# OpenResearchInstitute/opv-cxx-demod

Hardware: AMD Instinct MI355X
Metric: IQ Msamples/s demod+Viterbi (×real-time @2.168MSPS); BER vs ref (higher is better)
Workload: dtype f64; 1 GPU; configs[3]: 64 concurrent IQ streams/GPU x 1000 frames, -s semantics, amp 2000, f0 -2000..+2000 Hz across the 64 streams of a shard (SURVEY.md §8d C4: edge streams on the AFC clamp, outside the +/-1530 Hz search span), Eb/N0 16 dB; streams_per_gpu=64, parallelism=streams sharded 64/GPU, no data-path collective

## Files before the change

### opv-cxx-demod_amd/csrc/k_frontend.hip

```cpp
#include <hip/hip_runtime.h>
#include <math.h>

#include <type_traits>

#include "opv_device.h"

namespace {

constexpr double kPi = 3.14159265358979323846;
constexpr double kTwoPi = 2.0 * kPi;
constexpr double kFs = 2168000.0;
constexpr double kSymRate = 2168000.0 / 40.0;
constexpr double kDeltaPerHz = kTwoPi / kFs;

constexpr uint32_t kTile = OPV_TILE_SAMPLES;
constexpr uint32_t kRing = 2 * kTile;
constexpr uint32_t kRingBytes = kRing * 4;
constexpr uint32_t kGuardBytes = 16;
constexpr uint32_t kBack = 11;
constexpr uint32_t kAhead = 56;
static_assert((kRing & (kRing - 1)) == 0, "ring must be a power of two");

constexpr uint32_t kTabOff = kRingBytes + kGuardBytes;
static_assert(kTabOff % 16 == 0, "16-byte LDS alignment");

typedef __attribute__((address_space(1))) double gdouble;
typedef __attribute__((address_space(1))) unsigned char gbyte;

__device__ inline int dlo(double v) { return __double2loint(v); }
__device__ inline int dhi(double v) { return __double2hiint(v); }
__device__ inline double mkd(int hi, int lo) { return __hiloint2double(hi, lo); }

__device__ inline double swap32_add(double a, double b) {
    auto lo = __builtin_amdgcn_permlane32_swap((unsigned)dlo(a), (unsigned)dlo(b), false, false);
    auto hi = __builtin_amdgcn_permlane32_swap((unsigned)dhi(a), (unsigned)dhi(b), false, false);
    return mkd((int)hi[0], (int)lo[0]) + mkd((int)hi[1], (int)lo[1]);
}
__device__ inline double swap16_add(double a, double b) {
    auto lo = __builtin_amdgcn_permlane16_swap((unsigned)dlo(a), (unsigned)dlo(b), false, false);
    auto hi = __builtin_amdgcn_permlane16_swap((unsigned)dhi(a), (unsigned)dhi(b), false, false);
    return mkd((int)hi[0], (int)lo[0]) + mkd((int)hi[1], (int)lo[1]);
}
template <int N>
__device__ inline double row_bcast(double old, double v) { return __builtin_amdgcn_update_dpp(old, v, 0x150 + N, 0xF, 0xF, false); }
__device__ inline uint32_t uni(uint32_t v) { return (uint32_t)__builtin_amdgcn_readfirstlane((int)v); }
__device__ inline double readlane_d(double v, int l) {
    return mkd(__builtin_amdgcn_readlane(dhi(v), l), __builtin_amdgcn_readlane(dlo(v), l));
}
__device__ inline bool uni_lt(double a, double b) { return __builtin_amdgcn_fcmp(a, b, 4 ) != 0ull; }
__device__ inline bool uni_eq(double a, double b) { return __builtin_amdgcn_fcmp(a, b, 1 ) != 0ull; }
// ... 45 lines not shown
    th -= kTwoPi * rint(th / kTwoPi);
    double sn, cs;
    sincos(th, &sn, &cs);
    const unsigned q = (unsigned)((dom1 ? (4u - (unsigned)(ksym & 3u)) : (unsigned)(ksym & 3u)) & 3u);
    double er2 = cs, ei2 = sn;
    if (q == 1u) { er2 = -sn; ei2 = cs; }
    else if (q == 2u) { er2 = -cs; ei2 = -sn; }
    else if (q == 3u) { er2 = sn; ei2 = -cs; }
    double vr = dr, vi = di;
    if (dom_zero) {
        const double jr = dom1 ? pi : -pi, ji = dom1 ? -pr : pr;
        vr = jr * prv.x40c - ji * prv.x40s;
        vi = jr * prv.x40s + ji * prv.x40c;
    }
    const double qr = vr * er2 + vi * ei2;
    const double qi = vi * er2 - vr * ei2;
    return make_double2((qr < 0.0 && qi < 0.0) ? kPi : 0.0, tie);
}

}

#include "opv_atan2.h"

template <int WPB>
__device__ __forceinline__ void msk_frontend_body(OpvStream* __restrict__ streams, OpvGlobalCfg cfg, int n_streams,
                                                  unsigned char* lds_all) {
    const int lane = threadIdx.x & 63;
    const int wave = WPB == 1 ? 0 : __builtin_amdgcn_readfirstlane((int)(threadIdx.x >> 6));
    const int sidx = (int)blockIdx.x * WPB + wave;
    const uint64_t dbg_t0 = __builtin_amdgcn_s_memtime(), dbg_r0 = __builtin_amdgcn_s_memrealtime();

    unsigned char* const lds = lds_all + wave * kTabOff;
    const unsigned char* ringb = lds;
    double* atab = reinterpret_cast<double*>(lds_all + WPB * kTabOff);
    if (sidx >= n_streams) return;
    OpvStream& st = streams[sidx];

    const int jsamp = lane - (lane >> 4) - ((lane & 15) == 15 ? 1 : 0);
    const double kf = (double)(jsamp - 10);
    const double kfs = kf * kDeltaPerHz;
    double wr[15], wi[15];
    {
        const int row = lane >> 4, t = lane & 15, u = t & 7;
        const bool is_p = u >= 6, imag = t >= 8;
        const int gate = (u < 2 || is_p) ? 1 : ((u & 1) ? 2 : 0);
        const bool tone2 = is_p ? false : (u < 2 ? u == 1 : u >= 4);
#pragma unroll
        for (int n = 0; n < 15; ++n) {
            const int i = 15 * row + n - 10 * gate;
            double sn, cs;
            sincospi((double)i / 80.0, &sn, &cs);
            const bool in = i >= 0 && i < 40;
            const double a = in ? cs : 0.0, b = in ? -sn : 0.0;
            double r_, i_;
            if (is_p) { r_ = (t == 6) ? a : (t == 15 ? b : 0.0); i_ = (t == 7) ? b : (t == 14 ? a : 0.0); }
            else if (!imag) { r_ = a; i_ = tone2 ? -b : b; }
            else { r_ = tone2 ? b : -b; i_ = a; }
// ... 15 lines not shown
    asm volatile("" : "+v"(kc_halfpi), "+v"(kc_32), "+v"(kc_m1_32), "+v"(kc_gain));
    const double kc_nfomax = __builtin_canonicalize(-kc_fomax), kc_ntfmax = __builtin_canonicalize(-kc_tfmax);
    kc_fomax = __builtin_canonicalize(kc_fomax);
    kc_tfmax = __builtin_canonicalize(kc_tfmax);
    double sx = 1.0, nsg = 1.0;
    asm volatile("" : "+v"(sx), "+v"(nsg));

    double fo = st.freq_offset, tf = st.timing_freq, mu = st.mu;
    PrevSums qp{st.p1r, st.p1i, st.p2r, st.p2i, st.x40c, st.x40s}, qq{0, 0, 0, 0, 1, 0};
    double fo_sum = st.fo_sum;
    uint32_t origin = uni((uint32_t)st.origin);
    const uint32_t n_avail = uni((uint32_t)st.n_avail);
    uint64_t n_soft = st.n_soft, total_samples = st.total_samples;
    uint32_t n_chunks = uni(st.n_chunks);
    int tail_done = (int)uni((uint32_t)st.tail_done);
    const int eof = (int)uni((uint32_t)st.eof);
    int overflow = (int)uni((uint32_t)st.overflow), stalled = 0;
    uint32_t edge_ties = uni(st.edge_ties);
    const uint64_t cap_soft = st.cap_soft;
    if (cap_soft > (1ull << 28)) overflow = 1;
    uint64_t soft_keep = st.trk_next >= 24 ? st.trk_next - 24 : 0;
    if (st.trk_state != 0 && st.trk_anchor < soft_keep) soft_keep = st.trk_anchor;
    const uint32_t soft_bmask = (uint32_t)(cap_soft * 8u - 1u) & ~7u;
    gbyte* const soft_base = (gbyte*)st.soft;
    const gbyte* iq_bytes = (const gbyte*)st.iq;
    const uint64_t n_bytes = (uint64_t)n_avail * 4u;

    auto glds16 = [&](const gbyte* gsrc, uint32_t lds_byte) {
        unsigned keep;
        asm volatile("s_mov_b32 %0, m0\n\ts_mov_b32 m0, %2\n\ts_nop 0\n\tglobal_load_lds_dwordx4 %1, off\n\ts_mov_b32 m0, %0"
                     : "=&s"(keep)
                     : "v"(gsrc), "s"(uni(lds_byte))
                     : "memory");
    };
    const uint32_t lds_base = uni((uint32_t)(uintptr_t)(__attribute__((address_space(3))) unsigned char*)lds);
    auto issue_tile = [&](uint32_t t) {
        const uint64_t base = (uint64_t)t * OPV_TILE_BYTES;
        const uint32_t slot = (t & 1u) * OPV_TILE_BYTES;
#pragma unroll
        for (int r = 0; r < 8; ++r) {
            const uint32_t in_tile = (uint32_t)r * 1024u + (uint32_t)lane * 16u;
            const uint64_t off = base + in_tile;
            if (off + 16u <= n_bytes) glds16(iq_bytes + off, lds_base + slot + (uint32_t)r * 1024u);
            else if (off < n_bytes) {
                for (uint32_t j = 0; off + 4u * j < n_bytes; ++j)
                    *reinterpret_cast<int*>(lds + slot + in_tile + 4u * j) = *reinterpret_cast<const __attribute__((address_space(1))) int*>(iq_bytes + off + 4u * j);
            }
        }
        if ((t & 1u) == 0u && lane == 0) {
            if (base + 16u <= n_bytes) glds16(iq_bytes + base, lds_base + kRingBytes);
            else
                for (uint32_t j = 0; base + 4u * j < n_bytes && j < 4u; ++j)
                    *reinterpret_cast<int*>(lds + kRingBytes + 4u * j) = *reinterpret_cast<const __attribute__((address_space(1))) int*>(iq_bytes + base + 4u * j);
        }
    };
    uint32_t t_lo = (origin >= kBack ? origin - kBack : 0u) / kTile;
    issue_tile(t_lo);
    issue_tile(t_lo + 1u);
    __builtin_amdgcn_s_waitcnt(0x0F70);
    bool evt_issue = true;
    uint32_t next_evt = (t_lo + 1u) * kTile + kBack;

    for (;;) {
        const uint32_t remaining = n_avail - origin;
        uint32_t N;
        bool last = false;
        if (cfg.streaming) {
            if (remaining >= OPV_CHUNK) N = OPV_CHUNK;
            else if (eof && !tail_done && remaining > 0) { N = remaining; last = true; }
            else { if (eof) tail_done = 1; break; }
        } else {
            if (!eof || tail_done) break;
            N = n_avail;
            last = true;
        }
        if (overflow) break;
        if ((n_soft - soft_keep) + (uint64_t)(N / 38u + 2u) > cap_soft) { stalled = 1; break; }

        const double Nd = (double)N;
        double pos = mu;
        const uint32_t soft_off0 = ((uint32_t)n_soft * 8u) & soft_bmask;
        uint32_t soft_off = soft_off0;
        asm volatile("" : "+v"(soft_off));

        auto housekeeping = [&](double at) {
            const uint32_t b = uni((uint32_t)at);
            const uint32_t gb = origin + b;
            while (gb >= next_evt) {
                if (evt_issue) {
                    issue_tile(t_lo + 2u);
                    ++t_lo;
                    evt_issue = false;
                    next_evt = (t_lo + 1u) * kTile - kAhead;
                } else {
                    __builtin_amdgcn_s_waitcnt(0x0F70);
                    evt_issue = true;
                    next_evt = (t_lo + 1u) * kTile + kBack;
                }
            }
            const int lim1 = (int)(next_evt - gb) - 2, lim2 = (int)N - 52 - (int)b;
            int lim = lim1 < lim2 ? lim1 : lim2;
            if (lim < 0) lim = 0;
            return ((uint32_t)lim * 1560u) >> 16;
        };

        int w0 = 0, w1 = 0;
        double f = 0.0;
        uint32_t tap_byte = 0;
        auto fetch_addr = [&](double at, bool clamp0) {
            double p = at + kf;
            if (clamp0) p = fmax(p, 0.0);
            const int idx = (int)p;
            f = __builtin_amdgcn_fract(p);
            tap_byte = (((uint32_t)idx + origin) << 2) & (kRingBytes - 4u);
        };
        auto fetch_read = [&]() {
            const int* tap = reinterpret_cast<const int*>(ringb + tap_byte);
            w0 = tap[0];
            w1 = tap[1];
        };
        auto fetch = [&](double at, bool clamp0) {
            fetch_addr(at, clamp0);
            fetch_read();
        };

        auto symbol_r = [&](auto tag, PrevSums& cur, const PrevSums& prv) {
            constexpr bool kFirst = decltype(tag)::first;
            constexpr bool kWide = decltype(tag)::wide;
            double xs, xc;
            if constexpr (kWide) {
                if (__builtin_expect(uni_lt(2000.0, fabs(fo)), 0)) sincos(kfs * fo, &xs, &xc);
                else expj_small(kfs, fo, sck, xs, xc);
            } else {
                expj_small(kfs, fo, sck, xs, xc);
            }
            __builtin_amdgcn_sched_barrier(0);
            const uint32_t my_soft_off = soft_off;
            uint32_t soft_off_next = soft_off + 8u;
            asm volatile("" : "+v"(soft_off_next));
            __builtin_amdgcn_sched_barrier(0);
            const int s0r = (int)(short)(w0 & 0xFFFF), s0i = w0 >> 16;
            const int d_r = (int)(short)(w1 & 0xFFFF) - s0r, d_i = (w1 >> 16) - s0i;
            const double lr = fma(f, (double)d_r, (double)s0r);
            const double li = fma(f, (double)d_i, (double)s0i);
            const double zr = fma(lr, xc, li * xs);
            const double zi = fma(li, xc, -(lr * xs));
            __builtin_amdgcn_sched_barrier(0);

            double acc0, acc1, v, t;
#define OPV_RB(N) "v_fmac_f64_dpp %[a0], %[zr], %[r" #N "] row_newbcast:" #N " row_mask:0xf bank_mask:0xf\n\t" \
                  "v_fmac_f64_dpp %[a1], %[zi], %[i" #N "] row_newbcast:" #N " row_mask:0xf bank_mask:0xf\n\t"
            asm("v_mov_b64 %[a0], 0\n\tv_mov_b64 %[a1], 0\n\t" OPV_RB(0) OPV_RB(1) OPV_RB(2) OPV_RB(3) OPV_RB(4) OPV_RB(5) OPV_RB(6) OPV_RB(7)
                : [a0] "=&v"(acc0), [a1] "=&v"(acc1)
                : [zr] "v"(zr), [zi] "v"(zi), [r0] "v"(wr[0]), [i0] "v"(wi[0]), [r1] "v"(wr[1]), [i1] "v"(wi[1]), [r2] "v"(wr[2]), [i2] "v"(wi[2]),
                  [r3] "v"(wr[3]), [i3] "v"(wi[3]), [r4] "v"(wr[4]), [i4] "v"(wi[4]), [r5] "v"(wr[5]), [i5] "v"(wi[5]),
                  [r6] "v"(wr[6]), [i6] "v"(wi[6]), [r7] "v"(wr[7]), [i7] "v"(wi[7]));
            __builtin_amdgcn_sched_barrier(0);
            soft_off = soft_off_next & soft_bmask;
            asm volatile("" : "+v"(soft_off));
            __builtin_amdgcn_sched_barrier(0);
            asm(OPV_RB(8) OPV_RB(9) OPV_RB(10) OPV_RB(11) OPV_RB(12) OPV_RB(13) OPV_RB(14)
                "v_add_f64 %[v], %[a0], %[a1]\n\t"
                "v_mov_b64 %[t], %[v]"
                : [a0] "+v"(acc0), [a1] "+v"(acc1), [v] "=&v"(v), [t] "=&v"(t)
                : [zr] "v"(zr), [zi] "v"(zi), [r8] "v"(wr[8]), [i8] "v"(wi[8]), [r9] "v"(wr[9]), [i9] "v"(wi[9]), [r10] "v"(wr[10]), [i10] "v"(wi[10]),
                  [r11] "v"(wr[11]), [i11] "v"(wi[11]), [r12] "v"(wr[12]), [i12] "v"(wi[12]), [r13] "v"(wr[13]), [i13] "v"(wi[13]),
                  [r14] "v"(wr[14]), [i14] "v"(wi[14]));
// ... 35 lines not shown
            if constexpr (!kFirst) {
                const double dr = fma(sg, P2o, P1o), di = fma(-sg, P4o, P3o);
                const double prs = fma(sg, prv.a, prv.b), pis = fma(sg, prv.c, -prv.d);
                const double ar = fma(dr, prs, di * pis), ai = fma(di, prs, -(dr * pis));
                cy = fma(ar, prv.x40c, ai * prv.x40s);
                cx = fma(ar, prv.x40s, -(ai * prv.x40c));
                __builtin_amdgcn_sched_barrier(0);
                ee = row_bcast<2>(sq, seln); el = row_bcast<3>(shv, seln);
                __builtin_amdgcn_sched_barrier(0);
                sx = mkd((dhi(cx) & (int)0x80000000) | (dhi(sx) & 0x7fffffff), dlo(sx));
                asm volatile("" : "+v"(sx));
                sum = fabs(cx) + fabs(cy); dif = fabs(cy) - fabs(cx);
                dm_ = sum + kc_tiny;
                if constexpr (WPB == 1) {
                    zmask = __builtin_amdgcn_fcmp(sum, 0.0, 1 );
                    asm volatile("" : "+s"(zmask));
                }
            } else {
                ee = row_bcast<2>(sq, seln); el = row_bcast<3>(shv, seln);
            }
            const double den = el + ee + kc_eps;

            double ted, h = 0;
            [[maybe_unused]] double2 c01{0, 0}, c23{0, 0}, c45{0, 0};
            if constexpr (kFirst) {
                double y = __builtin_amdgcn_rcp(den);
                const double num = el - ee;
                y = fma(fma(-den, y, 1.0), y, y);
                y = fma(fma(-den, y, 1.0), y, y);
                ted = num * y;
                ted = fma(fma(-den, ted, num), y, ted);
            } else {
                const double dm = dm_;
                const double tt = den * dm;
                double y = __builtin_amdgcn_rcp(tt);
                const double num = el - ee;
                y = fma(fma(-tt, y, 1.0), y, y);
                const double iden = y * dm, idm = y * den;
                const double ratio = dif * idm;
                const double kt = fma(ratio, kc_64, kc_magic);
                h = ratio;
                const unsigned char* rowb = reinterpret_cast<const unsigned char*>(atab) + ((unsigned)dlo(kt) << 5);
                const double2* trow = reinterpret_cast<const double2*>(rowb);
                c23 = trow[1]; c01 = trow[0];
                ted = num * iden;
                ted = fma(fma(-den, ted, num), iden, ted);
            }
            __builtin_amdgcn_sched_barrier(0);
            tf = clampd(fma(kc_beta, ted, tf), kc_ntfmax, kc_tfmax);
            const double adj = fma(kc_alpha, ted, tf);
            pos += 40.0 + adj;
            fetch_addr(pos, false);
            __builtin_amdgcn_sched_barrier(0);
            fetch_read();
            __builtin_amdgcn_sched_barrier(0);
            *(gdouble*)(soft_base + my_soft_off) = soft;
            if constexpr (!kFirst) {
                const double pd_off = fma(-sx, kc_halfpi, kc_halfpi);
                __builtin_amdgcn_sched_barrier(0);
                __builtin_amdgcn_s_waitcnt(0xC17F);
                __builtin_amdgcn_sched_barrier(0);
                pd = fma(c23.y, h, c23.x);
                pd = fma(pd, h, c01.y);
                pd = fma(pd, h, c01.x);
                pd = fma(sx, pd, pd_off);
                pd = mkd((dhi(pd) & 0x7fffffff) | (dhi(cy) & (int)0x80000000), dlo(pd));
                if (__builtin_expect(WPB == 1 ? zmask != 0ull : uni_eq(sum, 0.0), 0)) {
                    const double dr = fma(sg, P2o, P1o), di = fma(-sg, P4o, P3o);
                    const double2 sp = silence_pd(dr, di, prv, soft < 0.0, fo_sum, n_soft + (((my_soft_off - soft_off0) & soft_bmask) >> 3),
                                                  P1o, P2o, P3o, P4o);
                    pd = sp.x;
                    edge_ties += uni((uint32_t)sp.y);
                }
                const double fo_new = fma(kc_gain, pd, fo);
                asm("v_max_f64 %0, %1, %2\n\tv_min_f64 %0, %0, %3" : "=&v"(fo) : "v"(fo_new), "v"(kc_nfomax), "v"(kc_fomax));
            }
            fo_sum = fo_sum_next;
            cur.a = P1o; cur.b = P2o; cur.c = P3o; cur.d = P4o;
        };

        auto sym = [&](auto tag, PrevSums& cur, const PrevSums& prv) { symbol_r(tag, cur, prv); };

        if (uni_lt(pos + 40.0 + 10.0, Nd)) {
            (void)housekeeping(pos);
            fetch(pos, true);
            sym(TagFirst{}, qp, qp);
            if (__builtin_expect(uni_lt(2000.0, fabs(fo)), 0) && uni_lt(pos + 40.0 + 10.0, Nd)) {
                (void)housekeeping(pos);
                fetch(pos, false);
                sym(TagSecond{}, qq, qp);
                qp = qq;
            }
            while (uni_lt(pos + 40.0 + 10.0, Nd)) {
                uint32_t pairs = uni(housekeeping(pos)) >> 1;
                fetch(pos, false);
                for (uint32_t quads = pairs >> 1; quads != 0u; --quads) {
                    sym(TagSteady{}, qq, qp);
                    sym(TagSteady{}, qp, qq);
                    sym(TagSteady{}, qq, qp);
                    sym(TagSteady{}, qp, qq);
                }
                pairs &= 1u;
                for (; pairs != 0u; --pairs) {
                    sym(TagSteady{}, qq, qp);
                    sym(TagSteady{}, qp, qq);
                }
                sym(TagSteady{}, qq, qp);
                qp = qq;
            }
        }

        const uint32_t nsym_call = ((soft_off - soft_off0) & soft_bmask) >> 3;
        const uint32_t used = uni((uint32_t)pos);
        mu = pos - (double)used;
        const uint32_t leftover = N - used;
        if (lane == 0) {
            double* c = st.chunk_log + 5 * (size_t)(n_chunks % st.cap_chunks);
            c[0] = fo;
            c[1] = tf; c[2] = mu; c[3] = (double)leftover; c[4] = (double)nsym_call;
        }
        ++n_chunks;
        n_soft += nsym_call;
        total_samples += N;
        origin += (leftover > 0u && leftover < N) ? used : N;
        if (last) { tail_done = 1; break; }
    }

    if (lane == 0) {
        st.freq_offset = fo;
        st.p1r = qp.a; st.p1i = qp.b; st.p2r = qp.c; st.p2i = qp.d; st.x40c = qp.x40c; st.x40s = qp.x40s;
        st.fo_sum = fo_sum;
        st.edge_ties = edge_ties;
        st.timing_freq = tf; st.mu = mu;
        st.origin = origin; st.n_soft = n_soft; st.total_samples = total_samples;
        st.n_chunks = n_chunks; st.tail_done = tail_done; st.overflow = overflow;
        st.stalled = stalled;
        unsigned hw, xcc;
        asm volatile("s_getreg_b32 %0, hwreg(HW_REG_HW_ID)" : "=s"(hw));
        asm volatile("s_getreg_b32 %0, hwreg(HW_REG_XCC_ID)" : "=s"(xcc));
        st.dbg_hw_id = hw; st.dbg_xcc_id = xcc;
        st.dbg_cycles = __builtin_amdgcn_s_memtime() - dbg_t0;
        st.dbg_ticks = __builtin_amdgcn_s_memrealtime() - dbg_r0;
    }
}

constexpr uint32_t kAtanQBytes = 1025 * 32;
template <int NT>
__device__ __forceinline__ void load_atan_table_q(unsigned char* lds_tab) {
    double* atab = reinterpret_cast<double*>(lds_tab);
    for (int i = threadIdx.x; i < 1025 * 4; i += NT) atab[i] = (&kOpvAtanTabQ3R[0][0])[i];
}
extern "C" __global__ __launch_bounds__(64) void k_msk_frontend_rb(OpvStream* __restrict__ streams, OpvGlobalCfg cfg,
                                                                    int n_streams) {
    __shared__ __attribute__((aligned(16))) unsigned char lds_all[kTabOff + kAtanQBytes];
    load_atan_table_q<64>(lds_all + kTabOff);
    __syncthreads();
    msk_frontend_body<1>(streams, cfg, n_streams, lds_all);
}
extern "C" __global__ __launch_bounds__(256) void k_msk_frontend_rb_wg4(OpvStream* __restrict__ streams, OpvGlobalCfg cfg,
                                                                         int n_streams) {
    __shared__ __attribute__((aligned(16))) unsigned char lds_all[4 * kTabOff + kAtanQBytes];
    load_atan_table_q<256>(lds_all + 4 * kTabOff);
    __syncthreads();
    msk_frontend_body<4>(streams, cfg, n_streams, lds_all);
}
```

### opv-cxx-demod_amd/csrc/opv_capi.hip

```cpp
#include <hip/hip_runtime.h>
#include <dlfcn.h>

#include <atomic>

#include <climits>
#include <cstddef>
#include <cmath>
#include <cstdio>
#include <cstdlib>
#include <cstring>
#include <new>
#include <string>
#include <thread>
#include <vector>

#include "../../include/opv_demod.h"
#include "opv_device.h"
#include "opv_offset_host.h"
#include "opv_tx_internal.h"

extern "C" __global__ void k_offset_search(OpvStream*, OpvGlobalCfg, const double*, uint32_t*);
extern "C" __global__ void k_tie_collect(const OpvStream*, const uint32_t*, uint32_t, uint32_t, uint32_t, OpvTieStage*);
extern "C" __global__ void k_tie_apply(OpvStream*, const OpvTieStage*, uint32_t, int);
extern "C" __global__ void k_msk_frontend_rb(OpvStream*, OpvGlobalCfg, int);
// ... 159 lines not shown
    static constexpr int kInSlots = 4;
    StreamIn* h_in = nullptr;
    hipEvent_t in_ev[kInSlots] = {};
    int* h_stall = nullptr;
    hipEvent_t done_ev = nullptr;
    unsigned round_no = 0;
    std::vector<OpvStream> mirror;
    std::vector<OpvStream> initial;
    std::vector<HostStream> hs;
    double* d_soft = nullptr;
    OpvFrameRec* d_frec = nullptr;
    OpvEventRec* d_events = nullptr;
    double* d_chunks = nullptr;
    uint8_t* d_frames = nullptr;
    int32_t* d_metrics = nullptr;
    double* d_fscale = nullptr;
    int32_t* d_counts = nullptr;
    double* d_offs_wtab = nullptr;
    uint32_t* d_tie_list = nullptr;
    bool host_ties = false;
    bool tx_trust_libm = false;
    bool push_gather = true;
    uint32_t push_gather_blocks = 32;
    struct TieWork {
        OpvTieStage* stage = nullptr;
        uint32_t slots = 0;
        std::atomic<uint64_t> decided{0};
        std::atomic<uint64_t> left{0};
    } tie;
    std::vector<int> search_now;
    void* h_bulk_tab = nullptr;
    size_t bulk_tab_bytes = 0;
    bool push_pending = false;
    hipEvent_t push_ev = nullptr;
    uint64_t cap_soft = 0;
    uint32_t cap_frames = 0, cap_events = 0, cap_chunks = 0;
    bool mirror_valid = false;
    bool maybe_stalled = false;
    double* d_tx_ckpt = nullptr;
    size_t tx_ckpt_cap = 0, tx_ckpt_have = 0;
    double* d_tx_phases = nullptr;
    size_t tx_phases_cap = 0, tx_phases_have = 0;
    uint8_t* d_tx_frames = nullptr;
    uint8_t* d_tx_codes = nullptr;
    uint8_t* d_tx_fpar = nullptr;
    size_t tx_frames_cap = 0;
// ... 78 lines not shown
}

extern "C" const char* opv_last_error(void) { return g_err.c_str(); }
extern "C" int opv_abi_version(void) { return OPV_ABI_VERSION; }

extern "C" int opv_create(opv_ctx** out, int n_streams, const opv_cfg* cfg) {
    if (!out || !cfg || n_streams <= 0 || cfg->max_samples == 0) return fail(OPV_EINVAL, "opv_create: bad arguments");
    if (cfg->max_samples >= (1ull << 31)) return fail(OPV_EINVAL, "opv_create: max_samples must be < 2^31");
    if ((cfg->have_init_offset && !std::isfinite(cfg->init_offset_hz)) || !std::isfinite(cfg->afc_alpha) || (cfg->coherent && !std::isfinite(cfg->pll_bw_hz)))
        return fail(OPV_EINVAL, "opv_create: init_offset_hz / afc_alpha / pll_bw_hz must be finite");
    int ndev = 0;
    if (hipGetDeviceCount(&ndev) != hipSuccess || ndev <= 0) return fail(OPV_ENODEV, "no HIP device visible");
    if (cfg->device < 0 || cfg->device >= ndev) return fail(OPV_ENODEV, "opv_cfg.device out of range");
    HIPCHK(hipSetDevice(cfg->device));
    hipDeviceProp_t prop;
    HIPCHK(hipGetDeviceProperties(&prop, cfg->device));
    if (std::strncmp(prop.gcnArchName, "gfx950", 6) != 0)
        return fail(OPV_ENODEV, "device is not gfx950 (MI355X); this library carries gfx950 code objects only");

    opv_ctx* c = new (std::nothrow) opv_ctx();
    if (!c) return fail(OPV_ENOMEM, "host allocation failed");
    c->n_streams = n_streams;
    c->cfg = *cfg;
    c->hs.resize(n_streams);
    c->mirror.resize(n_streams);

    const uint64_t M = cfg->max_samples;
    c->cap_soft = 1;
    while (c->cap_soft < M / 38 + 4096) c->cap_soft <<= 1;
    c->cap_frames = (uint32_t)(M / (uint64_t)(OPV_FSYMS * 38) + 4);
    c->cap_events = 4 * c->cap_frames + 64;
    c->cap_chunks = (uint32_t)(M / 80000 + 4);

    auto cleanup = [&](int code) { opv_destroy(c); return code; };
#define HIPCHK_C(expr)                                                        \
    do {                                                                      \
        hipError_t _e = (expr);                                               \
        if (_e != hipSuccess) return cleanup(fail(_e == hipErrorOutOfMemory ? OPV_ENOMEM : OPV_EHIP, #expr, _e)); \
    } while (0)

    HIPCHK_C(hipStreamCreateWithFlags(&c->stream, hipStreamNonBlocking));
    {
        int least = 0, greatest = 0;
        if (hipDeviceGetStreamPriorityRange(&least, &greatest) != hipSuccess ||
            hipStreamCreateWithPriority(&c->copy_stream, hipStreamNonBlocking, greatest) != hipSuccess) {
            (void)hipGetLastError();
// ... 15 lines not shown
    HIPCHK_C(hipMalloc(&c->d_chunks, sizeof(double) * 5 * c->cap_chunks * S));
    HIPCHK_C(hipMalloc(&c->d_frames, (size_t)OPV_FB * c->cap_frames * S));
    HIPCHK_C(hipMalloc(&c->d_metrics, sizeof(int32_t) * c->cap_frames * S));
    HIPCHK_C(hipMalloc(&c->d_fscale, sizeof(double) * c->cap_frames * S));
    HIPCHK_C(hipMalloc(&c->d_counts, sizeof(int32_t) * S));
    {
        std::vector<double> w((size_t)OPV_SPS * 2 * OPV_OFFS_TERMS);
        for (int i = 0; i < OPV_SPS; ++i) {
            const double u = (double)i - 19.5, cs = std::cos(M_PI * i / 80.0), sn = std::sin(M_PI * i / 80.0);
            double t = 1.0;
            for (int k = 0; k < OPV_OFFS_TERMS; ++k) {
                w[((size_t)i * 2 + 0) * OPV_OFFS_TERMS + k] = cs * t;
                w[((size_t)i * 2 + 1) * OPV_OFFS_TERMS + k] = sn * t;
                t = t * u / (double)(k + 1);
            }
        }
        HIPCHK_C(hipMalloc(&c->d_offs_wtab, sizeof(double) * w.size()));
        HIPCHK_C(hipMemcpy(c->d_offs_wtab, w.data(), sizeof(double) * w.size(), hipMemcpyHostToDevice));
    }
    c->host_ties = opv_offset_host_libm_matches_reference() && !std::getenv("OPV_OFFSET_DISTRUST_LIBM");
    c->tx_trust_libm = libm_flat_tops_as_assumed() && !std::getenv("OPV_TX_DISTRUST_LIBM");
    c->push_gather = !std::getenv("OPV_PUSH_NO_GATHER");
    if (const char* e = std::getenv("OPV_PUSH_GATHER_BLOCKS")) { const int v = atoi(e); if (v > 0) c->push_gather_blocks = (uint32_t)v; }
    if (c->host_ties) {
        HIPCHK_C(hipMalloc(&c->d_tie_list, sizeof(uint32_t) * (S + 1)));
        c->tie.slots = (uint32_t)(S < (size_t)OPV_TIE_SLOTS_MAX ? S : (size_t)OPV_TIE_SLOTS_MAX);
        if (hipHostMalloc((void**)&c->tie.stage, offsetof(OpvTieStage, slot) + sizeof(OpvTieSlot) * c->tie.slots, hipHostMallocDefault) != hipSuccess) {
            (void)hipGetLastError();
            c->tie.stage = nullptr;
            c->host_ties = false;
        } else {
            c->tie.stage->n = c->tie.stage->listed = c->tie.stage->beyond = 0;
        }
    }
    HIPCHK_C(hipMemsetAsync(c->d_frames, 0, (size_t)OPV_FB * c->cap_frames * S, c->stream));
    HIPCHK_C(hipMemsetAsync(c->d_counts, 0, sizeof(int32_t) * S, c->stream));
    k_fill_i32<<<256, 256, 0, c->stream>>>(c->d_metrics, INT32_MIN, (size_t)c->cap_frames * S);

    for (size_t i = 0; i < S; ++i) {
        OpvStream s;
        std::memset(&s, 0, sizeof s);
        s.soft = c->d_soft + c->cap_soft * i;
        s.cap_soft = c->cap_soft;
        s.frec = c->d_frec + (size_t)c->cap_frames * i;
        s.events = c->d_events + (size_t)c->cap_events * i;
        s.chunk_log = c->d_chunks + (size_t)5 * c->cap_chunks * i;
// ... 357 lines not shown
            }
            k_tie_apply<<<K, 192, 0, c->stream>>>(c->d_streams, c->tie.stage, K, S);
        }
    }
    if (tm) HIPCHK(hipEventRecord(c->ev[2], c->stream));
    const bool x4 = c->frontend == 4 || (c->frontend == 0 && S >= kFrontendX4MinStreams);
    if (c->cfg.coherent && !c->cfg.streaming) {
        const double wn = c->cfg.pll_bw_hz * 2.0 * M_PI, zeta = 0.707, fsym = 2168000.0 / 40.0;
        c->last_frontend = "k_coherent_frontend";
        k_coherent_frontend<<<S, 64, 0, c->stream>>>(c->d_streams, 2.0 * zeta * wn / fsym, wn * wn / (fsym * fsym));
    }
    else if (c->frontend == 16 || (c->frontend == 0 && S > kFrontendX16MinStreams)) {
        if (S > kFrontendX16Wg8MinStreams) { c->last_frontend = "k_msk_frontend_x16_wg8"; k_msk_frontend_x16_wg8<<<(S + 127) / 128, 512, 0, c->stream>>>(c->d_streams, g, S); }
        else if (S > 16) { c->last_frontend = "k_msk_frontend_x16_wg4"; k_msk_frontend_x16_wg4<<<(S + 63) / 64, 256, 0, c->stream>>>(c->d_streams, g, S); }
        else { c->last_frontend = "k_msk_frontend_x16"; k_msk_frontend_x16<<<1, 64, 0, c->stream>>>(c->d_streams, g, S); }
    }
    else if (x4) {
        c->last_frontend = "k_msk_frontend_x4_wg4";
        k_msk_frontend_x4_wg4<<<(S + 15) / 16, 256, 0, c->stream>>>(c->d_streams, g, S);
    }
    else if (S > kFrontendWg4MinStreams) {
        c->last_frontend = "k_msk_frontend_rb_wg4";
        k_msk_frontend_rb_wg4<<<(S + 3) / 4, 256, 0, c->stream>>>(c->d_streams, g, S);
    } else {
        c->last_frontend = "k_msk_frontend_rb";
        k_msk_frontend_rb<<<S, 64, 0, c->stream>>>(c->d_streams, g, S);
    }
    if (tm) { HIPCHK(hipEventRecord(c->ev[3], c->stream)); HIPCHK(hipEventRecord(c->ev[4], c->stream)); }
    k_sync_track<<<S, 64, 0, c->stream>>>(c->d_streams);
    if (tm) { HIPCHK(hipEventRecord(c->ev[5], c->stream)); HIPCHK(hipEventRecord(c->ev[6], c->stream)); }
    if (fr * (uint64_t)S <= kScaleWaveMaxFrames) k_frame_scale_wave<<<(unsigned)(fr * (uint64_t)S), 64, 0, c->stream>>>(c->d_streams, (uint32_t)fr);
    else k_frame_scale<<<(unsigned)((fr * (uint64_t)S + 63) / 64), 64, 0, c->stream>>>(c->d_streams, (uint32_t)fr, (uint32_t)S);
    k_frame_decode<<<(unsigned)(((fr + 1) / 2) * (uint64_t)S), 64, 0, c->stream>>>(c->d_streams, (uint32_t)((fr + 1) / 2));
    if (tm) { HIPCHK(hipEventRecord(c->ev[7], c->stream)); c->timing_valid = true; }
    k_collect_counts<<<(S + 63) / 64, 64, 0, c->stream>>>(c->d_streams, c->d_counts, S, c->h_stall + slot);
    HIPCHK(hipEventRecord(c->done_ev, c->stream));
    HIPCHK(hipGetLastError());
    return OPV_OK;
}

extern "C" int opv_set_frontend(opv_ctx* c, int streams_per_wave) {
    if (!c) return fail(OPV_EINVAL, "null context");
    if (streams_per_wave != 0 && streams_per_wave != 1 && streams_per_wave != 4 && streams_per_wave != 16)
        return fail(OPV_EINVAL, "opv_set_frontend: 0 (automatic), 1, 4 or 16 streams per wave");
    c->frontend = streams_per_wave;
    return OPV_OK;
}

extern "C" const char* opv_frontend_kernel(opv_ctx* c) { return c ? c->last_frontend : ""; }
// ... 213 lines not shown
    if (int r = check_stream(c, s)) return r;
    if (!out134) return fail(OPV_EINVAL, "null out");
    if (int r = c->refresh()) return r;
    std::memcpy(out134, c->mirror[s].energies, sizeof(double) * 134);
    return OPV_OK;
}

extern "C" int opv_offset_ties_on_host(opv_ctx* c) { return c && c->host_ties ? 1 : 0; }
extern "C" uint64_t opv_offset_ties_decided_on_host(opv_ctx* c) { return c ? c->tie.decided.load(std::memory_order_relaxed) : 0; }
extern "C" uint64_t opv_offset_ties_left_to_device(opv_ctx* c) { return c ? c->tie.left.load(std::memory_order_relaxed) : 0; }

extern "C" int opv_tap_wave_info(opv_ctx* c, int s, uint64_t out[4]) {
    if (int r = check_stream(c, s)) return r;
    if (!out) return fail(OPV_EINVAL, "null out");
    if (int r = c->refresh()) return r;
    const OpvStream& st = c->mirror[s];
    out[0] = st.dbg_hw_id; out[1] = st.dbg_xcc_id; out[2] = st.dbg_cycles; out[3] = st.dbg_ticks;
    return OPV_OK;
}

extern "C" int opv_tap_occupancy(opv_ctx* c, int out[6]) {
    if (!c || !out) return fail(OPV_EINVAL, "null argument");
    HIPCHK(hipSetDevice(c->cfg.device));
    const struct { const void* k; int threads; } ks[6] = {
        {(const void*)k_msk_frontend_rb, 64}, {(const void*)k_msk_frontend_rb_wg4, 256}, {(const void*)k_msk_frontend_x16_wg4, 256},
        {(const void*)k_msk_frontend_x4_wg4, 256}, {(const void*)k_frame_decode, 64}, {(const void*)k_frame_scale, 64}};
    for (int i = 0; i < 6; ++i) HIPCHK(hipOccupancyMaxActiveBlocksPerMultiprocessor(&out[i], ks[i].k, ks[i].threads, 0));
    return OPV_OK;
}

extern "C" int opv_decode_payloads(opv_ctx* c, const double* soft, size_t n, uint8_t* out, int32_t* metrics,
                                   int8_t* q, int8_t* deint, uint8_t* bits) {
    if (!c || !soft || !out || !metrics) return fail(OPV_EINVAL, "null argument");
    if (n == 0) return OPV_OK;
    HIPCHK(hipSetDevice(c->cfg.device));
    double* d_soft = nullptr;
    uint8_t* d_out = nullptr;
    int32_t* d_met = nullptr;
    int8_t *d_q = nullptr, *d_d = nullptr;
    uint8_t* d_b = nullptr;
    double* d_scale = nullptr;
    int rc = OPV_OK;
    auto chk = [&](hipError_t e, const char* w) { if (e != hipSuccess && rc == OPV_OK) rc = fail(OPV_EHIP, w, e); };
    chk(hipMalloc(&d_soft, sizeof(double) * OPV_CODED * n), "hipMalloc soft");
    chk(hipMalloc(&d_out, (size_t)OPV_FB * n), "hipMalloc out");
    chk(hipMalloc(&d_met, sizeof(int32_t) * n), "hipMalloc metrics");
    chk(hipMalloc(&d_scale, sizeof(double) * n), "hipMalloc scales");
    if (q) chk(hipMalloc(&d_q, (size_t)OPV_CODED * n), "hipMalloc q");
    if (deint) chk(hipMalloc(&d_d, (size_t)OPV_CODED * n), "hipMalloc deint");
    if (bits) chk(hipMalloc(&d_b, (size_t)OPV_FBITS * n), "hipMalloc bits");
// ... 336 lines not shown
```

### opv-cxx-demod_amd/csrc/opv_device.h

```cpp
#pragma once
#include <stdint.h>

#define OPV_SPS 40
#define OPV_SYNC_BITS 24
#define OPV_FB 134
#define OPV_FBITS 1072
#define OPV_CODED 2144
#define OPV_FSYMS 2168
#define OPV_CHUNK 86720
#define OPV_SYNC_WORD 0x02B8DBu

#define OPV_OFFS_TERMS 10

#define OPV_TILE_SAMPLES 2048
#define OPV_TILE_BYTES (OPV_TILE_SAMPLES * 4)

struct OpvFrameRec {
    uint64_t payload_sym;
    uint64_t release_sym;
    double quality;
    int32_t sync_ok;
    int32_t pad;
};

struct OpvEventRec {
    int32_t kind;
    int32_t count;
    uint64_t sym_idx;
    double corr;
    double raw;
};

struct OpvStream {
    const int16_t* iq;
    uint64_t n_avail;
    int32_t eof;
    int32_t pad0;
    double* soft;
// ... 77 lines not shown
```

Baseline: 8143 Msamples/s.

## Add helper-wave fp64 pre-converted LDS ring for single-stream frontend

For the single-wave-per-stream frontend, the launch becomes a 128-thread block in which a second helper wave streams int16 IQ from global memory, converts each sample and its forward difference to fp64 pairs, and writes them into a 2048-entry LDS ring. The demod wave waits on LDS flags instead of issuing global-to-LDS tile loads, and its per-symbol interpolation drops the unpack and int-to-double conversions in favour of reading two double2 values. The intent is to move decode work off the serial critical path of the demod wave. The cost is a larger LDS footprint, spin-wait producer/consumer synchronisation with timeout fallbacks that set overflow, and a switch to dynamic LDS with a fixed base offset.

```diff
diff --git a/opv-cxx-demod_amd/csrc/k_frontend.hip b/opv-cxx-demod_amd/csrc/k_frontend.hip
--- a/opv-cxx-demod_amd/csrc/k_frontend.hip
+++ b/opv-cxx-demod_amd/csrc/k_frontend.hip
@@ -23,9 +23,28 @@
 
 constexpr uint32_t kTabOff = kRingBytes + kGuardBytes;
 static_assert(kTabOff % 16 == 0, "16-byte LDS alignment");
+constexpr uint32_t kAtanQBytes = 1025 * 32;
+constexpr uintptr_t kRbLdsBase = 16;
+static_assert(kRbLdsBase + kTabOff + kAtanQBytes == OPV_RB_LDS_I16, "launch size of the int16-ring shape");
+
+constexpr uint32_t kF64Ring = 2048;
+constexpr uint32_t kF64RingBytes = kF64Ring * 32;
+constexpr uint32_t kF64Chunk = 256;
+constexpr uint32_t kF64TabOff = 0;
+constexpr uint32_t kF64RingOff = kAtanQBytes;
+constexpr uint32_t kF64FlagOff = kF64RingOff + kF64RingBytes;
+constexpr uint32_t kF64WaitSpins = 1u << 22;
+constexpr uint32_t kHelperSpins = 1u << 22;
+static_assert(kRbLdsBase + kF64FlagOff + 16 == OPV_RB_LDS_F64, "launch size of the fp64-ring shape");
+static_assert(kF64Ring % kF64Chunk == 0 && (kF64Ring & (kF64Ring - 1)) == 0, "chunks tile the power-of-two ring");
 
 typedef __attribute__((address_space(1))) double gdouble;
 typedef __attribute__((address_space(1))) unsigned char gbyte;
+typedef double d2v __attribute__((ext_vector_type(2)));
+typedef __attribute__((address_space(3))) unsigned char lbyte;
+typedef __attribute__((address_space(3))) int lint;
+typedef __attribute__((address_space(3))) double ldouble;
+typedef __attribute__((address_space(3))) d2v ld2v;
 
 __device__ inline int dlo(double v) { return __double2loint(v); }
 __device__ inline int dhi(double v) { return __double2hiint(v); }
@@ -117,17 +136,62 @@
 
 #include "opv_atan2.h"
 
-template <int WPB>
+typedef __attribute__((address_space(3))) volatile uint32_t lds_flag;
+__device__ inline lds_flag* f64_flags(lbyte* lds_all) {
+    return reinterpret_cast<lds_flag*>(lds_all + kF64FlagOff);
+}
+
+__device__ void f64_ring_helper(const OpvStream& st, lbyte* lds_all) {
+    const uint32_t lane = threadIdx.x & 63u;
+    lds_flag* const fl = f64_flags(lds_all);
+    const uint32_t n_avail = uni((uint32_t)st.n_avail), origin = uni((uint32_t)st.origin);
+    const int* const iq = reinterpret_cast<const int*>(st.iq);
+    uint32_t fill = ((origin >= kBack ? origin - kBack : 0u) / kF64Chunk) * kF64Chunk;
+    const uint32_t fill_end = n_avail + kAhead + 2u;
+    uint32_t spins = 0;
+    while ((int)(fill - fill_end) < 0) {
+        if (fl[2] != 0u) return;
+        if ((int)(fl[0] + kF64Ring - fill - kF64Chunk) < 0) {
+            if (++spins > kHelperSpins) return;
+            __builtin_amdgcn_s_sleep(8);
+            continue;
+        }
+        spins = 0;
+        const uint32_t n = fill + 4u * lane;
+        int w[5];
+        if (n + 4u <= n_avail) {
+            const int4 v = *reinterpret_cast<const int4*>(iq + n);
+            w[0] = v.x; w[1] = v.y; w[2] = v.z; w[3] = v.w;
+        } else {
+#pragma unroll
+            for (uint32_t k = 0; k < 4u; ++k) w[k] = n + k < n_avail ? iq[n + k] : 0;
+        }
+        w[4] = n + 4u < n_avail ? iq[n + 4u] : 0;
+#pragma unroll
+        for (int k = 0; k < 4; ++k) {
+            const int xr = (int)(short)(w[k] & 0xFFFF), xi = w[k] >> 16;
+            const int yr = (int)(short)(w[k + 1] & 0xFFFF) - xr, yi = (w[k + 1] >> 16) - xi;
+            ld2v* e = reinterpret_cast<ld2v*>(lds_all + kF64RingOff + (((n + (uint32_t)k) & (kF64Ring - 1u)) << 5));
+            e[0] = d2v{(double)xr, (double)xi};
+            e[1] = d2v{(double)yr, (double)yi};
+        }
+        __builtin_amdgcn_fence(__ATOMIC_RELEASE, "workgroup");
+        fill += kF64Chunk;
+        if (lane == 0u) fl[1] = fill;
+    }
+}
+
+template <int WPB, bool F64 = false>
 __device__ __forceinline__ void msk_frontend_body(OpvStream* __restrict__ streams, OpvGlobalCfg cfg, int n_streams,
-                                                  unsigned char* lds_all) {
+                                                  lbyte* lds_all) {
     const int lane = threadIdx.x & 63;
     const int wave = WPB == 1 ? 0 : __builtin_amdgcn_readfirstlane((int)(threadIdx.x >> 6));
     const int sidx = (int)blockIdx.x * WPB + wave;
     const uint64_t dbg_t0 = __builtin_amdgcn_s_memtime(), dbg_r0 = __builtin_amdgcn_s_memrealtime();
 
-    unsigned char* const lds = lds_all + wave * kTabOff;
-    const unsigned char* ringb = lds;
-    double* atab = reinterpret_cast<double*>(lds_all + WPB * kTabOff);
+    lbyte* const lds = lds_all + (F64 ? kF64RingOff : wave * kTabOff);
+    const lbyte* ringb = lds;
+    const ldouble* atab = reinterpret_cast<const ldouble*>(lds_all + (F64 ? kF64TabOff : WPB * kTabOff));
     if (sidx >= n_streams) return;
     OpvStream& st = streams[sidx];
 
@@ -189,7 +253,7 @@
     uint64_t soft_keep = st.trk_next >= 24 ? st.trk_next - 24 : 0;
     if (st.trk_state != 0 && st.trk_anchor < soft_keep) soft_keep = st.trk_anchor;
     const uint32_t soft_bmask = (uint32_t)(cap_soft * 8u - 1u) & ~7u;
-    gbyte* const soft_base = (gbyte*)st.soft;
+    gbyte* const soft_base = (gbyte*)(((uint64_t)uni((uint32_t)((uint64_t)st.soft >> 32)) << 32) | uni((uint32_t)(uint64_t)st.soft));
     const gbyte* iq_bytes = (const gbyte*)st.iq;
     const uint64_t n_bytes = (uint64_t)n_avail * 4u;
 
@@ -200,7 +264,7 @@
                      : "v"(gsrc), "s"(uni(lds_byte))
                      : "memory");
     };
-    const uint32_t lds_base = uni((uint32_t)(uintptr_t)(__attribute__((address_space(3))) unsigned char*)lds);
+    const uint32_t lds_base = uni((uint32_t)(uintptr_t)lds);
     auto issue_tile = [&](uint32_t t) {
         const uint64_t base = (uint64_t)t * OPV_TILE_BYTES;
         const uint32_t slot = (t & 1u) * OPV_TILE_BYTES;
@@ -211,22 +275,34 @@
             if (off + 16u <= n_bytes) glds16(iq_bytes + off, lds_base + slot + (uint32_t)r * 1024u);
             else if (off < n_bytes) {
                 for (uint32_t j = 0; off + 4u * j < n_bytes; ++j)
-                    *reinterpret_cast<int*>(lds + slot + in_tile + 4u * j) = *reinterpret_cast<const __attribute__((address_space(1))) int*>(iq_bytes + off + 4u * j);
+                    *reinterpret_cast<lint*>(lds + slot + in_tile + 4u * j) = *reinterpret_cast<const __attribute__((address_space(1))) int*>(iq_bytes + off + 4u * j);
             }
         }
         if ((t & 1u) == 0u && lane == 0) {
             if (base + 16u <= n_bytes) glds16(iq_bytes + base, lds_base + kRingBytes);
             else
                 for (uint32_t j = 0; base + 4u * j < n_bytes && j < 4u; ++j)
-                    *reinterpret_cast<int*>(lds + kRingBytes + 4u * j) = *reinterpret_cast<const __attribute__((address_space(1))) int*>(iq_bytes + base + 4u * j);
+                    *reinterpret_cast<lint*>(lds + kRingBytes + 4u * j) = *reinterpret_cast<const __attribute__((address_space(1))) int*>(iq_bytes + base + 4u * j);
         }
     };
     uint32_t t_lo = (origin >= kBack ? origin - kBack : 0u) / kTile;
-    issue_tile(t_lo);
-    issue_tile(t_lo + 1u);
-    __builtin_amdgcn_s_waitcnt(0x0F70);
+    if constexpr (!F64) {
+        issue_tile(t_lo);
+        issue_tile(t_lo + 1u);
+        __builtin_amdgcn_s_waitcnt(0x0F70);
+    }
     bool evt_issue = true;
     uint32_t next_evt = (t_lo + 1u) * kTile + kBack;
+    [[maybe_unused]] lds_flag* const fl = f64_flags(lds_all);
+    [[maybe_unused]] auto f64_wait = [&](uint32_t need) {
+        uint32_t r = uni(fl[1]);
+        for (uint32_t spins = 0; (int)(r - need) < 0;) {
+            if (overflow != 0 || ++spins > kF64WaitSpins) { overflow = 2; break; }
+            __builtin_amdgcn_s_sleep(1);
+            r = uni(fl[1]);
+        }
+        return r;
+    };
 
     for (;;) {
         const uint32_t remaining = n_avail - origin;
@@ -253,7 +329,14 @@
         auto housekeeping = [&](double at) {
             const uint32_t b = uni((uint32_t)at);
             const uint32_t gb = origin + b;
-            while (gb >= next_evt) {
+            if constexpr (F64) {
+                if (lane == 0) fl[0] = gb >= kBack ? gb - kBack : 0u;
+                uint32_t ready = uni(fl[1]);
+                if ((int)(ready - gb) < (int)(kAhead + 2u)) ready = f64_wait(gb + kAhead + 2u);
+                asm volatile("" ::: "memory");
+                next_evt = ready - kAhead;
+            }
+            while (!F64 && gb >= next_evt) {
                 if (evt_issue) {
                     issue_tile(t_lo + 2u);
                     ++t_lo;
@@ -272,6 +355,7 @@
         };
 
         int w0 = 0, w1 = 0;
+        [[maybe_unused]] d2v x0{0.0, 0.0}, dx{0.0, 0.0};
         double f = 0.0;
         uint32_t tap_byte = 0;
         auto fetch_addr = [&](double at, bool clamp0) {
@@ -279,12 +363,19 @@
             if (clamp0) p = fmax(p, 0.0);
             const int idx = (int)p;
             f = __builtin_amdgcn_fract(p);
-            tap_byte = (((uint32_t)idx + origin) << 2) & (kRingBytes - 4u);
+            if constexpr (F64) tap_byte = (((uint32_t)idx + origin) << 5) & (kF64RingBytes - 32u);
+            else tap_byte = (((uint32_t)idx + origin) << 2) & (kRingBytes - 4u);
         };
         auto fetch_read = [&]() {
-            const int* tap = reinterpret_cast<const int*>(ringb + tap_byte);
-            w0 = tap[0];
-            w1 = tap[1];
+            if constexpr (F64) {
+                const ld2v* tap = reinterpret_cast<const ld2v*>(ringb + tap_byte);
+                x0 = tap[0];
+                dx = tap[1];
+            } else {
+                const lint* tap = reinterpret_cast<const lint*>(ringb + tap_byte);
+                w0 = tap[0];
+                w1 = tap[1];
+            }
         };
         auto fetch = [&](double at, bool clamp0) {
             fetch_addr(at, clamp0);
@@ -306,10 +397,16 @@
             uint32_t soft_off_next = soft_off + 8u;
             asm volatile("" : "+v"(soft_off_next));
             __builtin_amdgcn_sched_barrier(0);
-            const int s0r = (int)(short)(w0 & 0xFFFF), s0i = w0 >> 16;
-            const int d_r = (int)(short)(w1 & 0xFFFF) - s0r, d_i = (w1 >> 16) - s0i;
-            const double lr = fma(f, (double)d_r, (double)s0r);
-            const double li = fma(f, (double)d_i, (double)s0i);
+            double lr, li;
+            if constexpr (F64) {
+                lr = fma(f, dx.x, x0.x);
+                li = fma(f, dx.y, x0.y);
+            } else {
+                const int s0r = (int)(short)(w0 & 0xFFFF), s0i = w0 >> 16;
+                const int d_r = (int)(short)(w1 & 0xFFFF) - s0r, d_i = (w1 >> 16) - s0i;
+                lr = fma(f, (double)d_r, (double)s0r);
+                li = fma(f, (double)d_i, (double)s0i);
+            }
             const double zr = fma(lr, xc, li * xs);
             const double zi = fma(li, xc, -(lr * xs));
             __builtin_amdgcn_sched_barrier(0);
@@ -391,7 +488,7 @@
             const double den = el + ee + kc_eps;
 
             double ted, h = 0;
-            [[maybe_unused]] double2 c01{0, 0}, c23{0, 0}, c45{0, 0};
+            [[maybe_unused]] d2v c01{0, 0}, c23{0, 0};
             if constexpr (kFirst) {
                 double y = __builtin_amdgcn_rcp(den);
                 const double num = el - ee;
@@ -409,8 +506,8 @@
                 const double ratio = dif * idm;
                 const double kt = fma(ratio, kc_64, kc_magic);
                 h = ratio;
-                const unsigned char* rowb = reinterpret_cast<const unsigned char*>(atab) + ((unsigned)dlo(kt) << 5);
-                const double2* trow = reinterpret_cast<const double2*>(rowb);
+                const lbyte* rowb = reinterpret_cast<const lbyte*>(atab) + ((unsigned)dlo(kt) << 5);
+                const ld2v* trow = reinterpret_cast<const ld2v*>(rowb);
                 c23 = trow[1]; c01 = trow[0];
                 ted = num * iden;
                 ted = fma(fma(-den, ted, num), iden, ted);
@@ -427,7 +524,8 @@
             if constexpr (!kFirst) {
                 const double pd_off = fma(-sx, kc_halfpi, kc_halfpi);
                 __builtin_amdgcn_sched_barrier(0);
-                __builtin_amdgcn_s_waitcnt(0xC17F);
+                if constexpr (F64) __builtin_amdgcn_s_waitcnt(0xC27F);
+                else __builtin_amdgcn_s_waitcnt(0xC17F);
                 __builtin_amdgcn_sched_barrier(0);
                 pd = fma(c23.y, h, c23.x);
                 pd = fma(pd, h, c01.y);
@@ -462,6 +560,7 @@
             }
             while (uni_lt(pos + 40.0 + 10.0, Nd)) {
                 uint32_t pairs = uni(housekeeping(pos)) >> 1;
+                if (F64 && overflow != 0) break;
                 fetch(pos, false);
                 for (uint32_t quads = pairs >> 1; quads != 0u; --quads) {
                     sym(TagSteady{}, qq, qp);
@@ -495,6 +594,9 @@
         if (last) { tail_done = 1; break; }
     }
 
+    if constexpr (F64) {
+        if (lane == 0) fl[2] = 1u;
+    }
     if (lane == 0) {
         st.freq_offset = fo;
         st.p1r = qp.a; st.p1i = qp.b; st.p2r = qp.c; st.p2i = qp.d; st.x40c = qp.x40c; st.x40s = qp.x40s;
@@ -513,23 +615,39 @@
     }
 }
 
-constexpr uint32_t kAtanQBytes = 1025 * 32;
 template <int NT>
-__device__ __forceinline__ void load_atan_table_q(unsigned char* lds_tab) {
-    double* atab = reinterpret_cast<double*>(lds_tab);
+__device__ __forceinline__ void load_atan_table_q(lbyte* lds_tab) {
+    ldouble* atab = reinterpret_cast<ldouble*>(lds_tab);
     for (int i = threadIdx.x; i < 1025 * 4; i += NT) atab[i] = (&kOpvAtanTabQ3R[0][0])[i];
 }
-extern "C" __global__ __launch_bounds__(64) void k_msk_frontend_rb(OpvStream* __restrict__ streams, OpvGlobalCfg cfg,
-                                                                    int n_streams) {
-    __shared__ __attribute__((aligned(16))) unsigned char lds_all[kTabOff + kAtanQBytes];
-    load_atan_table_q<64>(lds_all + kTabOff);
-    __syncthreads();
-    msk_frontend_body<1>(streams, cfg, n_streams, lds_all);
+extern "C" __global__ __launch_bounds__(128) void k_msk_frontend_rb(OpvStream* __restrict__ streams, OpvGlobalCfg cfg,
+                                                                     int n_streams) {
+    lbyte* const lds_dyn = reinterpret_cast<lbyte*>(kRbLdsBase);
+    if (blockDim.x == 128) {
+        load_atan_table_q<128>(lds_dyn + kF64TabOff);
+        if (threadIdx.x == 0) {
+            __attribute__((address_space(3))) uint32_t* const fl = reinterpret_cast<__attribute__((address_space(3))) uint32_t*>(lds_dyn + kF64FlagOff);
+            fl[0] = 0u;
+            fl[1] = 0u;
+            fl[2] = 0u;
+        }
+        __syncthreads();
+        if (__builtin_amdgcn_readfirstlane((int)(threadIdx.x >> 6)) != 0) {
+            if ((int)blockIdx.x < n_streams) f64_ring_helper(streams[blockIdx.x], lds_dyn);
+            return;
+        }
+        msk_frontend_body<1, true>(streams, cfg, n_streams, lds_dyn);
+    } else {
+        load_atan_table_q<64>(lds_dyn + kTabOff);
+        __syncthreads();
+        msk_frontend_body<1>(streams, cfg, n_streams, lds_dyn);
+    }
 }
 extern "C" __global__ __launch_bounds__(256) void k_msk_frontend_rb_wg4(OpvStream* __restrict__ streams, OpvGlobalCfg cfg,
                                                                          int n_streams) {
     __shared__ __attribute__((aligned(16))) unsigned char lds_all[4 * kTabOff + kAtanQBytes];
-    load_atan_table_q<256>(lds_all + 4 * kTabOff);
+    lbyte* const lds = (lbyte*)lds_all;
+    load_atan_table_q<256>(lds + 4 * kTabOff);
     __syncthreads();
-    msk_frontend_body<4>(streams, cfg, n_streams, lds_all);
-}
+    msk_frontend_body<4>(streams, cfg, n_streams, lds);
+}
diff --git a/opv-cxx-demod_amd/csrc/opv_capi.hip b/opv-cxx-demod_amd/csrc/opv_capi.hip
--- a/opv-cxx-demod_amd/csrc/opv_capi.hip
+++ b/opv-cxx-demod_amd/csrc/opv_capi.hip
@@ -205,6 +205,8 @@
     bool tx_trust_libm = false;
     bool push_gather = true;
     uint32_t push_gather_blocks = 32;
+    bool rb_fp64_ring = true;
+    int n_cu = 0;
     struct TieWork {
         OpvTieStage* stage = nullptr;
         uint32_t slots = 0;
@@ -329,6 +331,7 @@
     if (!c) return fail(OPV_ENOMEM, "host allocation failed");
     c->n_streams = n_streams;
     c->cfg = *cfg;
+    c->n_cu = prop.multiProcessorCount;
     c->hs.resize(n_streams);
     c->mirror.resize(n_streams);
 
@@ -390,6 +393,13 @@
     c->tx_trust_libm = libm_flat_tops_as_assumed() && !std::getenv("OPV_TX_DISTRUST_LIBM");
     c->push_gather = !std::getenv("OPV_PUSH_NO_GATHER");
     if (const char* e = std::getenv("OPV_PUSH_GATHER_BLOCKS")) { const int v = atoi(e); if (v > 0) c->push_gather_blocks = (uint32_t)v; }
+    c->rb_fp64_ring = !std::getenv("OPV_FRONTEND_INT16_RING");
+    {
+        hipFuncAttributes fa;
+        HIPCHK_C(hipFuncGetAttributes(&fa, (const void*)k_msk_frontend_rb));
+        if (fa.sharedSizeBytes != 0) return cleanup(fail(OPV_EHIP, "k_msk_frontend_rb was built with static LDS"));
+    }
+    if (c->rb_fp64_ring) HIPCHK_C(hipFuncSetAttribute((const void*)k_msk_frontend_rb, hipFuncAttributeMaxDynamicSharedMemorySize, OPV_RB_LDS_F64));
     if (c->host_ties) {
         HIPCHK_C(hipMalloc(&c->d_tie_list, sizeof(uint32_t) * (S + 1)));
         c->tie.slots = (uint32_t)(S < (size_t)OPV_TIE_SLOTS_MAX ? S : (size_t)OPV_TIE_SLOTS_MAX);
@@ -793,9 +803,12 @@
     else if (S > kFrontendWg4MinStreams) {
         c->last_frontend = "k_msk_frontend_rb_wg4";
         k_msk_frontend_rb_wg4<<<(S + 3) / 4, 256, 0, c->stream>>>(c->d_streams, g, S);
+    } else if (c->rb_fp64_ring && S <= c->n_cu) {
+        c->last_frontend = "k_msk_frontend_rb";
+        k_msk_frontend_rb<<<S, 128, OPV_RB_LDS_F64, c->stream>>>(c->d_streams, g, S);
     } else {
         c->last_frontend = "k_msk_frontend_rb";
-        k_msk_frontend_rb<<<S, 64, 0, c->stream>>>(c->d_streams, g, S);
+        k_msk_frontend_rb<<<S, 64, OPV_RB_LDS_I16, c->stream>>>(c->d_streams, g, S);
     }
     if (tm) { HIPCHK(hipEventRecord(c->ev[3], c->stream)); HIPCHK(hipEventRecord(c->ev[4], c->stream)); }
     k_sync_track<<<S, 64, 0, c->stream>>>(c->d_streams);
@@ -1055,10 +1068,10 @@
 extern "C" int opv_tap_occupancy(opv_ctx* c, int out[6]) {
     if (!c || !out) return fail(OPV_EINVAL, "null argument");
     HIPCHK(hipSetDevice(c->cfg.device));
-    const struct { const void* k; int threads; } ks[6] = {
-        {(const void*)k_msk_frontend_rb, 64}, {(const void*)k_msk_frontend_rb_wg4, 256}, {(const void*)k_msk_frontend_x16_wg4, 256},
-        {(const void*)k_msk_frontend_x4_wg4, 256}, {(const void*)k_frame_decode, 64}, {(const void*)k_frame_scale, 64}};
-    for (int i = 0; i < 6; ++i) HIPCHK(hipOccupancyMaxActiveBlocksPerMultiprocessor(&out[i], ks[i].k, ks[i].threads, 0));
+    const struct { const void* k; int threads; size_t lds; } ks[6] = {
+        {(const void*)k_msk_frontend_rb, 64, OPV_RB_LDS_I16}, {(const void*)k_msk_frontend_rb_wg4, 256, 0}, {(const void*)k_msk_frontend_x16_wg4, 256, 0},
+        {(const void*)k_msk_frontend_x4_wg4, 256, 0}, {(const void*)k_frame_decode, 64, 0}, {(const void*)k_frame_scale, 64, 0}};
+    for (int i = 0; i < 6; ++i) HIPCHK(hipOccupancyMaxActiveBlocksPerMultiprocessor(&out[i], ks[i].k, ks[i].threads, ks[i].lds));
     return OPV_OK;
 }
 
diff --git a/opv-cxx-demod_amd/csrc/opv_device.h b/opv-cxx-demod_amd/csrc/opv_device.h
--- a/opv-cxx-demod_amd/csrc/opv_device.h
+++ b/opv-cxx-demod_amd/csrc/opv_device.h
@@ -14,6 +14,8 @@
 
 #define OPV_TILE_SAMPLES 2048
 #define OPV_TILE_BYTES (OPV_TILE_SAMPLES * 4)
+#define OPV_RB_LDS_I16 (16 + 2 * OPV_TILE_BYTES + 16 + 1025 * 32)
+#define OPV_RB_LDS_F64 (16 + 1025 * 32 + 2048 * 32 + 16)
 
 struct OpvFrameRec {
     uint64_t payload_sym;
```

New measurement: 8698 Msamples/s (median of 6 runs). 1.07x the previous value.
